# EntityOfCode/eoc-tfhe

Measured on AMD Instinct MI355X. Metric: gate bootstraps/sec (HomNAND), higher is better.
Workload: dtype f64

## Files before the change

eoc_tfhe_amd/__init__.py:

```python
import ctypes as C
import os

import numpy as np

_HERE = os.path.dirname(os.path.abspath(__file__))
LIB_PATH = os.environ.get("EOC_TFHE_LIB") or os.path.join(_HERE, "libeoc_tfhe_gpu.so")
N = 1024

OPS = dict(NAND=0, AND=1, OR=2, NOR=3, XOR=4, XNOR=5, ANDNY=6, ANDYN=7, ORNY=8, ORYN=9,
           MUX=10, NOT=11, COPY=12, CONST0=13, CONST1=14,
           MAJ=15, XOR3=16)


class EocError(RuntimeError):
    pass


class Params(C.Structure):
    _fields_ = [("n", C.c_int32), ("l", C.c_int32), ("Bgbit", C.c_int32), ("ks_t", C.c_int32),
                ("ks_basebit", C.c_int32), ("ks_stdev", C.c_double), ("bk_stdev", C.c_double)]

    def copy(self):
        q = Params()
        C.memmove(C.byref(q), C.byref(self), C.sizeof(Params))
# ... 96 lines not shown
        "eoc_decrypt_ints": (C.c_int, [vp, C.c_int, vp, sz, vp]),
        "eoc_lut_test_polynomial": (C.c_int, [C.c_int, vp, vp]),
        "eoc_lut_batch": (C.c_int, [C.c_int, vp, sz, vp, vp, sz]),
        "eoc_lut_many_test_polynomial": (C.c_int, [C.c_int, C.c_int, vp, vp]),
        "eoc_lut_many_batch_device": (C.c_int, [vp, C.c_int, vp, sz, vp, vp, sz, vp]),
        "eoc_lut_many_batch": (C.c_int, [C.c_int, C.c_int, vp, sz, vp, vp, sz]),
        "eoc_global_encrypt_ints": (C.c_int, [C.c_int, vp, sz, vp]),
        "eoc_global_decrypt_ints": (C.c_int, [C.c_int, vp, sz, vp]),
        "eoc_engine_stats": (C.c_int, [vp, C.POINTER(u64 * 3)]),
        "eoc_stats": (C.c_int, [C.POINTER(u64 * 3)]),
        "eoc_gpu_init": (C.c_int, [C.c_int, PP]),
        "eoc_gpu_init_multi": (C.c_int, [vp, C.c_int, PP]),
        "eoc_gpu_init_from_env": (C.c_int, [PP]),
        "eoc_gpu_set_devices": (C.c_int, [C.POINTER(C.c_int), C.c_int]),
        "eoc_gpu_engine_count": (C.c_int, []),
        "eoc_global_engine_at": (vp, [C.c_int]),
        "eoc_upload_cloud_key_arrays": (C.c_int, [vp, vp]),
        "eoc_stats_multi": (C.c_int, [vp, C.c_int, C.POINTER(C.c_double)]),
        "eoc_key_broadcast_method": (C.c_char_p, []),
        "eoc_host_path_buffer_grows": (u64, []),
        "eoc_rccl_origin": (C.c_char_p, []),
        "eoc_rccl_selftest": (C.c_int, [C.c_int, sz]),
        "eoc_worker_wakeups": (u64, [C.c_int]),
        "eoc_shard_range": (None, [sz, C.c_int, C.c_int, C.POINTER(sz), C.POINTER(sz)]),
        "eoc_gate_batch_submit": (C.c_int, [C.c_int, vp, vp, vp, vp, vp, sz, C.POINTER(u64)]),
        "eoc_gate_batch_wait": (C.c_int, [u64]),
        "eoc_global_gate_batch_submit": (C.c_int, [C.c_int, vp, vp, vp, vp, vp, sz, C.POINTER(u64)]),
        "eoc_host_alloc": (vp, [sz]),
        "eoc_host_free": (None, [vp]),
        "eoc_engine_reserve": (C.c_int, [vp, sz, sz, sz]),
        "eoc_engine_workspace_grows": (u64, [vp]),
        "eoc_engine_blind_rotate_launches": (u64, [vp]),
        "eoc_engine_blind_rotate_wide_launches": (u64, [vp]),
        "eoc_engine_resident_jobs": (C.c_size_t, [vp]),
        "eoc_engine_device": (C.c_int, [vp]),
        "eoc_engine_params": (PP, [vp]),
        "eoc_engine_adopt_cloud_key_device": (C.c_int, [vp, vp, vp]),
        "eoc_upload_cloud_key": (C.c_int, [vp]),
        "eoc_global_engine": (vp, []),
        "eoc_gpu_shutdown": (None, []),
        "eoc_gate_batch": (C.c_int, [C.c_int, vp, vp, vp, vp, vp, sz]),
        "eoc_circuit_run": (C.c_int, [vp, sz, vp, sz, sz]),
        "generateGateKey": (vp, [C.c_int, u64]),
        "resetGateKey": (None, []),
        "encryptBit": (vp, [C.c_int, C.c_char_p]),
        "decryptBit": (C.c_int, [C.c_char_p, C.c_char_p]),
        "constantBit": (vp, [C.c_int]),
        "gateNAND": (vp, [C.c_char_p, C.c_char_p, C.c_char_p]),
        "gateAND": (vp, [C.c_char_p, C.c_char_p, C.c_char_p]),
        "gateOR": (vp, [C.c_char_p, C.c_char_p, C.c_char_p]),
        "gateNOR": (vp, [C.c_char_p, C.c_char_p, C.c_char_p]),
        "gateXOR": (vp, [C.c_char_p, C.c_char_p, C.c_char_p]),
        "gateXNOR": (vp, [C.c_char_p, C.c_char_p, C.c_char_p]),
        "gateNOT": (vp, [C.c_char_p, C.c_char_p]),
        "gateMUX": (vp, [C.c_char_p, C.c_char_p, C.c_char_p, C.c_char_p]),
        "gateMAJ": (vp, [C.c_char_p, C.c_char_p, C.c_char_p, C.c_char_p]),
        "gateXOR3": (vp, [C.c_char_p, C.c_char_p, C.c_char_p, C.c_char_p]),
        "generateSecretKey": (vp, [C.c_char_p, C.c_char_p]),
        "generatePublicKey": (vp, []),
        "encryptInteger": (vp, [C.c_int32, C.c_char_p]),
        "encryptInteger_dummy": (vp, [C.c_int32, C.c_char_p]),
        "decryptInteger": (C.c_int, [C.c_char_p, C.c_char_p, C.c_char_p, C.c_char_p]),
        "addCiphertexts": (vp, [C.c_char_p, C.c_char_p, C.c_char_p]),
        "subtractCiphertexts": (vp, [C.c_char_p, C.c_char_p, C.c_char_p]),
        "encrypt8BitASCIIString": (vp, [C.c_char_p, C.c_int16, C.c_char_p]),
        "decrypt8BitASCIIString": (vp, [C.c_char_p, C.c_int16, C.c_char_p, C.c_char_p, C.c_char_p]),
# ... 369 lines not shown
        _check(self.L.eoc_circuit_run_device(self.h, C.addressof(arr), len(gates), d_wires, n_wires, instances, stream),
               "eoc_circuit_run_device")

    def fft_fwd_device(self, d_polys, d_specs, count, stream=None):
        _check(self.L.eoc_dbg_fft_fwd_device(self.h, d_polys, d_specs, count, stream), "eoc_dbg_fft_fwd_device")

    def fft_inv_device(self, d_specs, d_polys, count, stream=None):
        _check(self.L.eoc_dbg_fft_inv_device(self.h, d_specs, d_polys, count, stream), "eoc_dbg_fft_inv_device")

    def blind_rotate_device(self, d_t, d_u, count, stream=None):
        _check(self.L.eoc_blind_rotate_device(self.h, d_t, d_u, count, stream), "eoc_blind_rotate_device")

    def keyswitch_device(self, d_u, d_out, count, stream=None):
        _check(self.L.eoc_keyswitch_device(self.h, d_u, d_out, count, stream), "eoc_keyswitch_device")

    def lut_batch_device(self, d_tv, n_luts, d_in, d_out, count, stream=None):
        _check(self.L.eoc_lut_batch_device(self.h, d_tv, n_luts, d_in, d_out, count, stream), "eoc_lut_batch_device")

    def lut_many_batch_device(self, n_tables, d_tv, n_luts, d_in, d_out, count, stream=None):
        _check(self.L.eoc_lut_many_batch_device(self.h, int(n_tables), d_tv, n_luts, d_in, d_out, count, stream),
               "eoc_lut_many_batch_device")

    def compact_expand_device(self, d_lists, count, d_out, stream=None):
        _check(self.L.eoc_compact_expand_device(self.h, d_lists, count, d_out, stream), "eoc_compact_expand_device")

    def resident_jobs(self):
        return int(self.L.eoc_engine_resident_jobs(self.h))

    def stats(self):
        out = (C.c_uint64 * 3)()
        _check(self.L.eoc_engine_stats(self.h, C.byref(out)), "eoc_engine_stats")
        return dict(batches=out[0], bootstraps=out[1], keyswitches=out[2],
                    br_launches=int(self.L.eoc_engine_blind_rotate_launches(self.h)),
                    br_wide_launches=int(self.L.eoc_engine_blind_rotate_wide_launches(self.h)))


def circuit_bootstraps(gates):
    arr = (Gate * len(gates))(*gates)
    return lib().eoc_circuit_bootstraps(C.addressof(arr), len(gates))


def netlist_optimize(gates, outputs, extension_gates=True):
    arr = (Gate * max(1, len(gates)))(*gates)
    out = (Gate * max(1, len(gates)))()
    outs = (C.c_int32 * max(1, len(outputs)))(*outputs)
    n = lib().eoc_netlist_optimize_ex(C.addressof(arr), len(gates), C.addressof(outs), len(outputs), C.addressof(out),
                                      0 if extension_gates else 1)
    if n < 0:
        raise EocError(f"eoc_netlist_optimize failed ({n}): not a single-assignment netlist?")
    return [Gate(out[k].op, out[k].in0, out[k].in1, out[k].in2, out[k].out) for k in range(n)]


def netlist_levels(gates):
    arr = (Gate * max(1, len(gates)))(*gates)
    lev = (C.c_int32 * max(1, len(gates)))()
    depth = C.c_int64(0)
    n = lib().eoc_netlist_levels(C.addressof(arr), len(gates), C.addressof(lev), C.addressof(depth))
    if n < 0:
        raise EocError(f"eoc_netlist_levels failed ({n})")
    return list(lev[:len(gates)]), int(n), int(depth.value)


def netlist_cost(gates, instances, resident_jobs=0):
    arr = (Gate * max(1, len(gates)))(*gates)
    c = lib().eoc_netlist_cost(C.addressof(arr), len(gates), int(instances), int(resident_jobs))
    if c < 0:
        raise EocError(f"eoc_netlist_cost failed ({c})")
# ... 511 lines not shown
```

eoc_tfhe_amd/csrc/engine.hip:

```cpp
#include "kernels.hip.h"
#include "canon_twiddles.h"
#include "common.h"
#include "../../include/eoc_tfhe_gpu.h"

#include <algorithm>
#include <cstdio>
#include <cstdlib>
#include <cstring>
#include <mutex>
#include <new>
#include <vector>

using namespace eoc;

#define HIP_TRY(expr)                                                                       \
    do {                                                                                    \
        hipError_t _e = (expr);                                                             \
        if (_e != hipSuccess) {                                                             \
            eoc_set_error("%s failed: %s (%s:%d)", #expr, hipGetErrorString(_e), __FILE__, \
                          __LINE__);                                                        \
            return EOC_ERR_HIP;                                                             \
        }                                                                                   \
    } while (0)

struct eoc_engine {
    int device = 0;
    eoc_params p{};
    int kpl = 0;
    size_t n1p = 0;
    d2 *d_tw = nullptr, *d_twist = nullptr;
    double *d_bkfft = nullptr;
    int32_t *d_ksk = nullptr;
    bool own_keys = false;
    const double *bkfft = nullptr;
    const int32_t *ksk = nullptr;
    struct Workspace {
        uint16_t *d_bara = nullptr;
        int32_t *d_u = nullptr;
        uint32_t *d_ubar = nullptr;
        int32_t *d_acc_state = nullptr;
        size_t ws_jobs = 0;
        GateDesc *d_descs = nullptr, *h_descs = nullptr;
        size_t ws_descs = 0, desc_pos = 0;
        hipEvent_t ring_ev = nullptr;
        bool ring_ev_set = false;
        bool ring_pushed_since_mark = false;
        GateDesc *d_persist = nullptr, *h_persist = nullptr;
        size_t persist_cap = 0, persist_pos = 0;
        int32_t *d_mixed = nullptr;
        uint32_t *h_perm = nullptr;
        hipEvent_t perm_ev = nullptr;
        size_t ws_mixed = 0;
    } ws;
    unsigned long long *d_stamps = nullptr;
    int num_cus = 256;
    int prio_duty_override = INT32_MIN;
    int prio_multi = -1;
    int br_slice = 0;
    bool no_fold = false;
    bool scalar_abar = false;
    bool no_pool = false;
    int br_parts = 0;
    int br_wide = -1;
    int bara_stride = 0;
    bool ks_waves_ok = true;
    uint64_t stats[3] = {0, 0, 0};
    uint64_t ws_grows = 0;
    uint64_t br_launches = 0;
    uint64_t br_wide_launches = 0;
    bool profiling = false;
    struct Span { hipEvent_t a, b; int kind; };
    std::vector<Span> spans;
    double kernel_ms[3] = {0, 0, 0};
    uint64_t kernel_launches[3] = {0, 0, 0};
    std::mutex mu;
};

enum { KIND_PREPARE = 0, KIND_BLIND_ROTATE = 1, KIND_KEYSWITCH = 2 };

struct SpanGuard {
    eoc_engine *e;
    hipStream_t st;
    hipEvent_t a = nullptr, b = nullptr;
    int kind;
    SpanGuard(eoc_engine *e_, hipStream_t st_, int kind_) : e(e_), st(st_), kind(kind_)
    {
        if (!e->profiling) return;
        if (hipEventCreate(&a) != hipSuccess || hipEventCreate(&b) != hipSuccess) {
            a = b = nullptr;
            return;
        }
        hipEventRecord(a, st);
    }
    ~SpanGuard()
    {
        if (!a) return;
        hipEventRecord(b, st);
        e->spans.push_back({a, b, kind});
    }
};

static int valid_params(const eoc_params *p)
// ... 86 lines not shown
                      "-- the FP64 external product is not exact beyond that --, ks_t * ks_basebit <= 31, ks_basebit <= 4)");
        return EOC_ERR_ARG;
    }
    int cnt = eoc_device_count();
    if (cnt <= 0 || device < 0 || device >= cnt) {
        eoc_set_error("eoc_engine_create: no usable HIP device (count=%d, asked %d); the gate path has no CPU fallback",
                      cnt, device);
        return EOC_ERR_NO_DEVICE;
    }
    HIP_TRY(hipSetDevice(device));
    eoc_engine *e = new (std::nothrow) eoc_engine();
    if (!e) return EOC_ERR_ALLOC;
    e->device = device;
    e->p = *p;
    e->kpl = 2 * p->l;
    e->n1p = eoc_ksk_row_stride(p);
    e->bara_stride = (p->n + 1 + 31) / 32 * 32;
    int rc = upload_tables(e);
    if (rc) {
        delete e;
        return rc;
    }
    {
        int cus = 0;
        if (hipDeviceGetAttribute(&cus, hipDeviceAttributeMultiprocessorCount, device) == hipSuccess && cus > 0) e->num_cus = cus;
        if (const char *s = getenv("EOC_TFHE_PRIO_DUTY")) e->prio_duty_override = atoi(s);
        if (const char *s = getenv("EOC_TFHE_PRIO_MULTI")) e->prio_multi = atoi(s);
        if (const char *s = getenv("EOC_TFHE_BR_SLICE")) e->br_slice = atoi(s);
        if (getenv("EOC_TFHE_NO_FOLD")) e->no_fold = true;
        if (getenv("EOC_TFHE_NO_POOL")) e->no_pool = true;
        if (const char *s = getenv("EOC_TFHE_SCALAR_ABAR")) e->scalar_abar = atoi(s) != 0;
        if (const char *s = getenv("EOC_TFHE_BR_PARTS")) e->br_parts = atoi(s);
        if (const char *s = getenv("EOC_TFHE_BR_WIDE")) e->br_wide = atoi(s);
    }
#define EOC_KS_ATTR(TT, NWV, IWV)                                                                              \
    if (hipFuncSetAttribute(reinterpret_cast<const void *>(&k_keyswitch_waves<TT, NWV, IWV>),                  \
                            hipFuncAttributeMaxDynamicSharedMemorySize, KS3Cfg<TT, NWV, IWV>::LDS_BYTES) != hipSuccess) \
        e->ks_waves_ok = false
    EOC_KS_ATTR(8, 8, 16);
    EOC_KS_ATTR(8, 8, 32);
    EOC_KS_ATTR(8, 4, 64);
    EOC_KS_ATTR(8, 8, 64);
#undef EOC_KS_ATTR
    if (!e->ks_waves_ok) (void)hipGetLastError();
    *out = e;
    return EOC_OK;
}

static void free_ws(eoc_engine::Workspace &W)
{
    hipFree(W.d_bara);
    hipFree(W.d_u);
    hipFree(W.d_ubar);
    hipFree(W.d_acc_state);
    hipFree(W.d_descs);
    hipFree(W.d_mixed);
    if (W.h_descs) hipHostFree(W.h_descs);
    if (W.h_perm) hipHostFree(W.h_perm);
    if (W.perm_ev) hipEventDestroy(W.perm_ev);
    if (W.ring_ev) hipEventDestroy(W.ring_ev);
    hipFree(W.d_persist);
    if (W.h_persist) hipHostFree(W.h_persist);
    W = eoc_engine::Workspace();
}

extern "C" void eoc_engine_destroy(eoc_engine *e)
{
    if (!e) return;
    hipSetDevice(e->device);
    hipDeviceSynchronize();
    hipFree(e->d_tw);
    hipFree(e->d_twist);
    if (e->own_keys) {
        hipFree(e->d_bkfft);
        hipFree(e->d_ksk);
    }
    free_ws(e->ws);
    hipFree(e->d_stamps);
    delete e;
}

static bool stream_is_capturing(hipStream_t st)
{
    hipStreamCaptureStatus cap = hipStreamCaptureStatusNone;
    return st && hipStreamIsCapturing(st, &cap) == hipSuccess && cap == hipStreamCaptureStatusActive;
}

static int ensure_ws(eoc_engine *e, eoc_engine::Workspace &W, size_t jobs, size_t descs, size_t mixed, hipStream_t st = nullptr)
{
    if (jobs <= W.ws_jobs && descs <= W.ws_descs && mixed <= W.ws_mixed) return EOC_OK;
    if (stream_is_capturing(st)) {
        eoc_set_error("graph capture: the workspace would have to grow (jobs %zu > %zu, descriptors %zu > %zu or mixed rows "
                      "%zu > %zu); call eoc_engine_reserve with the sizes of the captured work before capturing",
                      jobs, W.ws_jobs, descs, W.ws_descs, mixed, W.ws_mixed);
        return EOC_ERR_STATE;
    }
    HIP_TRY(hipDeviceSynchronize());
    if (jobs > W.ws_jobs) {
        hipFree(W.d_bara);
        hipFree(W.d_u);
        hipFree(W.d_ubar);
        W.d_bara = nullptr;
        W.d_u = nullptr;
        W.d_ubar = nullptr;
        W.ws_jobs = 0;
        size_t cap = (std::max<size_t>(jobs, 1024) + 63) / 64 * 64;
        HIP_TRY(hipMalloc(&W.d_bara, cap * e->bara_stride * sizeof(uint16_t)));
        HIP_TRY(hipMalloc(&W.d_u, cap * (kN + 1) * sizeof(int32_t)));
        HIP_TRY(hipMalloc(&W.d_ubar, (cap + KS_GT) * (size_t)kN * sizeof(uint32_t)));
// ... 114 lines not shown
    HIP_TRY(hipSetDevice(e->device));
    hipStream_t st = (hipStream_t)hip_stream;
    dim3 grid((unsigned)((count + 3) / 4));
    hipLaunchKernelGGL(k_fft_inv_polys, grid, dim3(256), 0, st, d_specs, d_polys, count, e->d_tw, e->d_twist);
    HIP_TRY(hipGetLastError());
    return EOC_OK;
}

static int build_cloud_key_images(eoc_engine *e, const int32_t *bk, const int32_t *ksk, double *d_bkfft,
                                  int32_t *d_ksk)
{
    const eoc_params &p = e->p;
    const size_t npoly = (size_t)p.n * e->kpl * 2;
    int32_t *d_bk = nullptr;
    HIP_TRY(hipMalloc(&d_bk, npoly * kN * 4));
    if (hipMemcpy(d_bk, bk, npoly * kN * 4, hipMemcpyHostToDevice) != hipSuccess) {
        hipFree(d_bk);
        eoc_set_error("cloud key upload failed");
        return EOC_ERR_HIP;
    }
    int rc = launch_fft_fwd(e, d_bk, d_bkfft, npoly, 0x1p-9, nullptr);
    hipError_t se = hipDeviceSynchronize();
    hipFree(d_bk);
    if (rc) return rc;
    HIP_TRY(se);
    const size_t rows = (size_t)kN * p.ks_t * (((size_t)1 << p.ks_basebit) - 1);
    HIP_TRY(hipMemset(d_ksk, 0, eoc_ksk_dev_bytes(&p)));
    HIP_TRY(hipMemcpy2D(d_ksk, e->n1p * 4, ksk, (size_t)(p.n + 1) * 4, (size_t)(p.n + 1) * 4, rows,
                        hipMemcpyHostToDevice));
    HIP_TRY(hipDeviceSynchronize());
    return EOC_OK;
}

extern "C" int eoc_engine_load_cloud_key(eoc_engine *e, const int32_t *bk, const int32_t *ksk)
{
    if (!e || !bk || !ksk) return EOC_ERR_ARG;
    std::lock_guard<std::mutex> g(e->mu);
    HIP_TRY(hipSetDevice(e->device));
    if (!e->own_keys) {
        HIP_TRY(hipMalloc(&e->d_bkfft, eoc_bkfft_bytes(&e->p)));
        HIP_TRY(hipMalloc(&e->d_ksk, eoc_ksk_dev_bytes(&e->p)));
        e->own_keys = true;
    }
    int rc = build_cloud_key_images(e, bk, ksk, e->d_bkfft, e->d_ksk);
    if (rc) return rc;
    e->bkfft = e->d_bkfft;
    e->ksk = e->d_ksk;
    return EOC_OK;
}

extern "C" int eoc_engine_build_cloud_key_device(eoc_engine *e, const int32_t *bk, const int32_t *ksk,
                                                 void *d_bkfft, void *d_ksk)
{
    if (!e || !bk || !ksk || !d_bkfft || !d_ksk) return EOC_ERR_ARG;
    std::lock_guard<std::mutex> g(e->mu);
    HIP_TRY(hipSetDevice(e->device));
    int rc = build_cloud_key_images(e, bk, ksk, static_cast<double *>(d_bkfft), static_cast<int32_t *>(d_ksk));
    if (rc) return rc;
    e->bkfft = static_cast<const double *>(d_bkfft);
    e->ksk = static_cast<const int32_t *>(d_ksk);
    return EOC_OK;
}

extern "C" int eoc_engine_set_cloud_key_device(eoc_engine *e, const void *d_bkfft, const void *d_ksk)
{
    if (!e || !d_bkfft || !d_ksk) return EOC_ERR_ARG;
    std::lock_guard<std::mutex> g(e->mu);
    e->bkfft = static_cast<const double *>(d_bkfft);
    e->ksk = static_cast<const int32_t *>(d_ksk);
    return EOC_OK;
}
extern "C" int eoc_engine_adopt_cloud_key_device(eoc_engine *e, void *d_bkfft, void *d_ksk)
{
    if (!e || !d_bkfft || !d_ksk) return EOC_ERR_ARG;
    std::lock_guard<std::mutex> g(e->mu);
    HIP_TRY(hipSetDevice(e->device));
    if (e->own_keys) {
        hipFree(e->d_bkfft);
        hipFree(e->d_ksk);
    }
    e->d_bkfft = static_cast<double *>(d_bkfft);
    e->d_ksk = static_cast<int32_t *>(d_ksk);
    e->own_keys = true;
    e->bkfft = e->d_bkfft;
    e->ksk = e->d_ksk;
    return EOC_OK;
}
extern "C" int eoc_engine_cloud_key_device(eoc_engine *e, const void **d_bkfft, const void **d_ksk)
{
    if (!e || !e->bkfft || !e->ksk) return EOC_ERR_NO_KEY;
    if (d_bkfft) *d_bkfft = e->bkfft;
    if (d_ksk) *d_ksk = e->ksk;
    return EOC_OK;
}

typedef eoc_engine::Workspace WS;

struct BRWork {
    uint32_t njobs = 0;
    enum Seed { GATE, TV, MANY } seed = GATE;
    const int32_t *tv = nullptr;
    uint32_t tv_rows = 1, n_tables = 0;
    enum Fold { NONE, KS, KS_AND_PREP } fold = NONE;
    const GateDesc *descs = nullptr, *inline_desc = nullptr;
    uint32_t S = 0;
};

struct BRSeg { uint32_t off, njobs; bool wide; };
struct BRPlan {
    std::vector<BRSeg> segs;
    int parts;
};
static BRPlan plan_blind_rotate(uint32_t njobs_total, int num_cus, int l, int kpl, int n, int br_slice, int br_parts, int br_wide)
{
    const uint32_t resident_pair = 4u * (uint32_t)num_cus, resident_wide = 8u * (uint32_t)num_cus;
    const bool can_wide = l == 2 && br_wide != 0;
    const bool force_wide = can_wide && br_wide > 0;
    const int auto_parts = kpl * 2 * kNH * 16 > 80 * 1024 ? 2 : 1;
    BRPlan plan;
// ... 79 lines not shown
    else if (l == 3 && Bgbit == 7) fn = br_pair_kernel<3, 7>(seed, sabar);
    else if (l == 1) fn = br_pair_kernel<1, 0>(seed, sabar);
    else if (l == 2) fn = br_pair_kernel<2, 0>(seed, sabar);
    else if (l == 3) fn = br_pair_kernel<3, 0>(seed, sabar);
    else if (l == 4) fn = br_pair_kernel<4, 0>(seed, sabar);
    return {fn, dim3(njobs), dim3(128), kBRLds};
}

static int launch_blind_rotate(eoc_engine *e, WS &W, const BRWork &w, hipStream_t st)
{
    const bool folds = w.fold != BRWork::NONE;
    if ((w.seed != BRWork::GATE && !w.tv) || (w.seed == BRWork::MANY && (folds || w.n_tables == 0)) ||
        (folds && !w.inline_desc && (!w.descs || !w.S)) || (w.inline_desc && (w.fold != BRWork::KS_AND_PREP || !w.S))) {
        eoc_set_error("internal: blind rotation of family %d with fold %d: a table family needs its test polynomials, the "
                      "many-LUT kernel has no fold, a fold needs descriptors and their row count", (int)w.seed, (int)w.fold);
        return EOC_ERR_STATE;
    }
    SpanGuard span(e, st, KIND_BLIND_ROTATE);
    const BRPlan plan = plan_blind_rotate(w.njobs, e->num_cus, e->p.l, e->kpl, e->p.n, e->br_slice, e->br_parts, e->br_wide);
    for (const BRSeg &sg : plan.segs) {
        const BRKernel k = blind_rotate_kernel(sg.wide, e->p.l, e->p.Bgbit, e->scalar_abar, w.seed, sg.njobs);
        if (!k.fn) return EOC_ERR_ARG;
        for (int part = 0; part < plan.parts; part++) {
            BRArgs a = blind_rotate_args(e, W, w, sg, part, plan.parts);
            void *args[] = {&a, (void *)&e->d_tw, (void *)&e->d_twist, (void *)&w.tv, (void *)&w.tv_rows, (void *)&w.n_tables};
            HIP_TRY(hipLaunchKernel(k.fn, k.grid, k.block, args, k.lds, st));
            e->br_launches++;
            e->br_wide_launches += sg.wide;
        }
    }
    return EOC_OK;
}

static int launch_keyswitch(eoc_engine *e, WS &W, const GateDesc *d_descs, uint32_t ngates, uint32_t S, hipStream_t st,
                            bool init_done, const GateDesc *inline_desc)
{
    KSArgs a;
    a.inline_desc = inline_desc != nullptr;
    if (inline_desc) a.desc0 = *inline_desc;
    else a.desc0 = GateDesc{0, 0, nullptr, nullptr, nullptr, nullptr};
    a.ksk = e->ksk;
    a.u = W.d_u;
    a.ubar = W.d_ubar;
    a.n = e->p.n;
    a.n1p = (int)e->n1p;
    a.t = e->p.ks_t;
    a.basebit = e->p.ks_basebit;
    a.S = S;
    a.mu = (int32_t)(1u << 29);
    SpanGuard span(e, st, KIND_KEYSWITCH);
    if (!init_done) {
        hipLaunchKernelGGL(k_ks_init, dim3(S, ngates), dim3(256), 0, st, d_descs, a);
        HIP_TRY(hipGetLastError());
    }
    const uint32_t ntiles = (S + KS_GT - 1) / KS_GT;
    const int ncb = (int)(e->n1p / 64);
    const int bb = e->p.ks_basebit, t = e->p.ks_t;
#define EOC_KS_LAUNCH(TT, NWV, IWV)                                                                     \
    do {                                                                                                  \
        auto kfn = k_keyswitch_waves<TT, NWV, IWV>;                                                       \
        constexpr int lds = KS3Cfg<TT, NWV, IWV>::LDS_BYTES;                                              \
        constexpr int ns = KS3Cfg<TT, NWV, IWV>::NS;                                                      \
        hipLaunchKernelGGL(kfn, dim3(ntiles * (unsigned)ncb * ns, ngates), dim3(64 * NWV), lds, st, d_descs, a); \
    } while (0)
    const bool fast = bb == 2 && t == 8 && e->ks_waves_ok;
    if (fast && ncb == 4) EOC_KS_LAUNCH(8, 8, 16);
    else if (fast && ncb == 8) EOC_KS_LAUNCH(8, 8, 32);
    else if (fast && ncb == 12) EOC_KS_LAUNCH(8, 4, 64);
    else if (fast && ncb == 16) EOC_KS_LAUNCH(8, 8, 64);
    else
        hipLaunchKernelGGL(k_keyswitch_generic, dim3(S, ngates), dim3(256), 0, st, d_descs, a);
#undef EOC_KS_LAUNCH
    HIP_TRY(hipGetLastError());
    return EOC_OK;
}

static inline bool op_const(int op) { return op == OP_CONST0 || op == OP_CONST1; }
static inline bool op_free(int op) { return op == OP_NOT || op == OP_COPY || op_const(op); }
static inline bool op_valid(int op) { return (op >= 0 && op <= OP_XOR3); }
static inline bool op_lin3(int op) { return op == OP_MAJ || op == OP_XOR3; }
static inline int op_inputs(int op) { return op_const(op) ? 0 : (op_free(op) ? 1 : (op == OP_MUX || op_lin3(op) ? 3 : 2)); }

constexpr size_t kMaxGatesPerLaunch = 32768;

static int push_descs(WS &W, const GateDesc *src, size_t count, hipStream_t st, GateDesc **d_out)
{
    if (stream_is_capturing(st)) {
        if (W.persist_pos + count > W.persist_cap) {
            eoc_set_error("graph capture: descriptor arena exhausted (%zu of %zu used, %zu wanted); "
                          "eoc_engine_reserve a larger max_descs before capturing", W.persist_pos, W.persist_cap, count);
            return EOC_ERR_STATE;
        }
        memcpy(W.h_persist + W.persist_pos, src, count * sizeof(GateDesc));
        HIP_TRY(hipMemcpyAsync(W.d_persist + W.persist_pos, W.h_persist + W.persist_pos, count * sizeof(GateDesc),
                               hipMemcpyHostToDevice, st));
        *d_out = W.d_persist + W.persist_pos;
        W.persist_pos += count;
        return EOC_OK;
    }
// ... 573 lines not shown
            e->kernel_ms[i] = 0;
            e->kernel_launches[i] = 0;
        }
    }
    return EOC_OK;
}

#ifdef EOC_STAMPS
extern "C" int eoc_dbg_stamps(eoc_engine *e, size_t waves, unsigned long long *host_out)
{
    if (!e) return EOC_ERR_ARG;
    HIP_TRY(hipSetDevice(e->device));
    if (!host_out) {
        hipFree(e->d_stamps);
        HIP_TRY(hipMalloc(&e->d_stamps, waves * 16 * 8));
        HIP_TRY(hipMemset(e->d_stamps, 0, waves * 16 * 8));
        return EOC_OK;
    }
    HIP_TRY(hipDeviceSynchronize());
    HIP_TRY(hipMemcpy(host_out, e->d_stamps, waves * 16 * 8, hipMemcpyDeviceToHost));
    return EOC_OK;
}
#endif

extern "C" int eoc_engine_stats(eoc_engine *e, uint64_t out[3])
{
    if (!e || !out) return EOC_ERR_ARG;
    for (int i = 0; i < 3; i++) out[i] = e->stats[i];
    return EOC_OK;
}
extern "C" uint64_t eoc_engine_workspace_grows(eoc_engine *e) { return e ? e->ws_grows : 0; }
extern "C" uint64_t eoc_engine_blind_rotate_launches(eoc_engine *e) { return e ? e->br_launches : 0; }
extern "C" uint64_t eoc_engine_blind_rotate_wide_launches(eoc_engine *e) { return e ? e->br_wide_launches : 0; }
extern "C" size_t eoc_engine_resident_jobs(eoc_engine *e)
{
    if (!e) return 0;
    const bool wide = e->p.l == 2 && e->br_wide != 0;
    return (size_t)(wide ? 8 : 4) * (size_t)e->num_cus;
}
extern "C" int eoc_engine_device(eoc_engine *e) { return e ? e->device : -1; }
extern "C" const eoc_params *eoc_engine_params(eoc_engine *e) { return e ? &e->p : nullptr; }
```

eoc_tfhe_amd/csrc/kernels.hip.h:

```cpp
#pragma once
#include <hip/hip_runtime.h>
#include <stdint.h>
#include <type_traits>

namespace eoc {

typedef double d2 __attribute__((ext_vector_type(2)));

constexpr int kN = 1024;
constexpr int kNH = 512;
constexpr int kScr = 568;
constexpr int kTwF1 = 0;
constexpr int kTwF2 = 32;
constexpr int kTwI1 = 32 + 256;
constexpr int kTwI0 = 32 + 256 + 32;
constexpr int kTwEntries = 32 + 256 + 32 + 256;

#define EOC_FMA(a, b, c) __builtin_fma((a), (b), (c))

#define EOC_SQRT_HALF 0x1.6a09e667f3bcdp-1
#define EOC_E128_RE 0x1.d906bcf328d46p-1
#define EOC_E128_IM 0x1.87de2a6aea963p-2
#define EOC_E64_RE 0x1.f6297cff75cb0p-1
#define EOC_E64_IM 0x1.8f8b83c69a60bp-3
// ... 863 lines not shown
        int *r = s_all + lane * C::ROWI;
#pragma unroll
        for (int c = 0; c < 16; c++) *reinterpret_cast<i4 *>(r + 4 * c) = acc[c];
    }
    __syncthreads();
    const int col = (int)cb * 64 + lane;
#pragma unroll 4
    for (int k = 0; k < 64 / NWV; k++) {
        const int ct = w * (64 / NWV) + k;
        const int v = s_all[ct * C::ROWI + lane];
        if (v != 0 && s0 + ct < A.S && col <= A.n) atomicAdd(d.out + (size_t)(s0 + ct) * (A.n + 1) + col, v);
    }
}

__global__ __launch_bounds__(256) void k_keyswitch_generic(const GateDesc *__restrict__ descs, KSArgs A)
{
    const GateDesc d = A.inline_desc ? A.desc0 : descs[blockIdx.y];
    const uint32_t s = blockIdx.x, job = d.job_base + s;
    const int base1 = (1 << A.basebit) - 1;
    int32_t *o = d.out + (size_t)s * (A.n + 1);
    for (int m = threadIdx.x; m <= A.n; m += 256) {
        uint32_t acc = (uint32_t)o[m];
        for (int i = 0; i < kN; i++) {
            const uint32_t ub = A.ubar[(size_t)job * kN + i];
            for (int j = 0; j < A.t; j++) {
                const uint32_t dg = (ub >> (32 - (j + 1) * A.basebit)) & (uint32_t)base1;
                if (dg) acc -= (uint32_t)A.ksk[(((size_t)i * A.t + j) * base1 + (dg - 1)) * A.n1p + m];
            }
        }
        o[m] = (int32_t)acc;
    }
}

constexpr int kCompactSlotsPerWG = 16;
__global__ __launch_bounds__(256) void k_compact_expand(const int32_t *__restrict__ lists, uint64_t first, uint32_t S,
                                                        uint32_t *__restrict__ ubar, int32_t *__restrict__ out, int n,
                                                        uint32_t prec_offset)
{
    static_assert(kN % kCompactSlotsPerWG == 0, "a workgroup's slots lie inside one list");
    __shared__ int32_t s_c0[kN];
    const uint64_t g0 = (first / kCompactSlotsPerWG + blockIdx.x) * kCompactSlotsPerWG;
    const int32_t *list = lists + (g0 / kN) * (uint64_t)(2 * kN);
    for (int k = threadIdx.x; k < kN; k += 256) s_c0[k] = list[k];
    __syncthreads();
    for (int q = 0; q < kCompactSlotsPerWG; q++) {
        const uint64_t g = g0 + q;
        if (g < first || g >= first + S) continue;
        const uint32_t s = (uint32_t)(g - first);
        const int j = (int)(g % kN);
        uint32_t *row = ubar + (size_t)s * kN;
        for (int i = threadIdx.x; i < kN; i += 256) {
            const uint32_t v = (uint32_t)s_c0[(j - i) & (kN - 1)];
            row[i] = (i <= j ? v : 0u - v) + prec_offset;
        }
        int32_t *o = out + (size_t)s * (n + 1);
        for (int m = threadIdx.x; m < n; m += 256) o[m] = 0;
        if (threadIdx.x == 0) o[n] = list[kN + j];
    }
}

}
```

include/eoc_tfhe_gpu.h:

```cpp
#ifndef EOC_TFHE_GPU_H
#define EOC_TFHE_GPU_H
#include <stddef.h>
#include <stdint.h>

#ifdef __cplusplus
extern "C" {
#endif

#define EOC_N 1024

typedef struct eoc_params {
    int32_t n;
    int32_t l;
    int32_t Bgbit;
    int32_t ks_t;
    int32_t ks_basebit;
    double ks_stdev;
    double bk_stdev;
} eoc_params;

enum eoc_op {
    EOC_NAND = 0, EOC_AND = 1, EOC_OR = 2, EOC_NOR = 3, EOC_XOR = 4, EOC_XNOR = 5,
    EOC_ANDNY = 6, EOC_ANDYN = 7, EOC_ORNY = 8, EOC_ORYN = 9, EOC_MUX = 10,
    EOC_NOT = 11, EOC_COPY = 12,
// ... 40 lines not shown
int32_t eoc_lwe_phase(const eoc_secret_key *sk, const int32_t *ct);
int eoc_host_threads(void);
int32_t eoc_modswitch_to_torus32(int32_t mu, int32_t Msize);
int32_t eoc_modswitch_from_torus32(int32_t phase, int32_t Msize);

typedef struct eoc_engine eoc_engine;

int eoc_device_count(void);
int eoc_engine_create(int device, const eoc_params *p, eoc_engine **out);
void eoc_engine_destroy(eoc_engine *e);
const char *eoc_last_error(void);

int eoc_device_alloc(eoc_engine *e, size_t bytes, void **d_ptr);
int eoc_device_free(eoc_engine *e, void *d_ptr);
int eoc_host_to_device(eoc_engine *e, void *d_dst, const void *src, size_t bytes);
int eoc_device_to_host(eoc_engine *e, void *dst, const void *d_src, size_t bytes);
int eoc_engine_synchronize(eoc_engine *e);

size_t eoc_bkfft_bytes(const eoc_params *p);
size_t eoc_ksk_dev_bytes(const eoc_params *p);
size_t eoc_ksk_row_stride(const eoc_params *p);

int eoc_engine_load_cloud_key(eoc_engine *e, const int32_t *bk, const int32_t *ksk);
int eoc_engine_build_cloud_key_device(eoc_engine *e, const int32_t *bk, const int32_t *ksk,
                                      void *d_bkfft, void *d_ksk);
int eoc_engine_set_cloud_key_device(eoc_engine *e, const void *d_bkfft, const void *d_ksk);
int eoc_engine_adopt_cloud_key_device(eoc_engine *e, void *d_bkfft, void *d_ksk);
int eoc_engine_cloud_key_device(eoc_engine *e, const void **d_bkfft, const void **d_ksk);

int eoc_engine_reserve(eoc_engine *e, size_t max_jobs, size_t max_descs, size_t max_mixed_rows);
uint64_t eoc_engine_workspace_grows(eoc_engine *e);
uint64_t eoc_engine_blind_rotate_launches(eoc_engine *e);
uint64_t eoc_engine_blind_rotate_wide_launches(eoc_engine *e);
size_t eoc_engine_resident_jobs(eoc_engine *e);
int eoc_engine_device(eoc_engine *e);
const eoc_params *eoc_engine_params(eoc_engine *e);
int eoc_gate_batch_device(eoc_engine *e, int op, const uint8_t *ops, const int32_t *d_in0,
                          const int32_t *d_in1, const int32_t *d_in2, int32_t *d_out, size_t count,
                          void *hip_stream);

typedef struct eoc_gate {
    int32_t op;
    int32_t in0, in1, in2;
    int32_t out;
} eoc_gate;
int eoc_circuit_run_device(eoc_engine *e, const eoc_gate *gates, size_t n_gates, int32_t *d_wires,
                           size_t n_wires, size_t instances, void *hip_stream);
size_t eoc_circuit_bootstraps(const eoc_gate *gates, size_t n_gates);
int64_t eoc_netlist_optimize(const eoc_gate *gates, size_t n_gates, const int32_t *outputs, size_t n_outputs,
                             eoc_gate *gates_out);
enum { EOC_NL_BOOTS_GATES_ONLY = 1 };
int64_t eoc_netlist_optimize_ex(const eoc_gate *gates, size_t n_gates, const int32_t *outputs, size_t n_outputs,
                                eoc_gate *gates_out, unsigned flags);
int64_t eoc_netlist_levels(const eoc_gate *gates, size_t n_gates, int32_t *level_of, int64_t *bootstrap_levels);
int64_t eoc_netlist_cost(const eoc_gate *gates, size_t n_gates, size_t instances, size_t resident_jobs);

int eoc_dbg_fft_fwd_device(eoc_engine *e, const int32_t *d_polys, double *d_specs, size_t count,
                           void *hip_stream);
int eoc_dbg_fft_inv_device(eoc_engine *e, const double *d_specs, int32_t *d_polys, size_t count,
                           void *hip_stream);
int eoc_blind_rotate_device(eoc_engine *e, const int32_t *d_t, int32_t *d_u, size_t count,
                            void *hip_stream);
int eoc_keyswitch_device(eoc_engine *e, const int32_t *d_u, int32_t *d_out, size_t count,
                         void *hip_stream);
int eoc_lut_batch_device(eoc_engine *e, const int32_t *d_tv, size_t n_luts, const int32_t *d_in, int32_t *d_out,
                         size_t count, void *hip_stream);
// ... 117 lines not shown
```

Baseline: 338,100.

## Add MFMA int8 keyswitch kernel using byte-limb decomposed key-switching key

```diff
diff --git a/eoc_tfhe_amd/__init__.py b/eoc_tfhe_amd/__init__.py
--- a/eoc_tfhe_amd/__init__.py
+++ b/eoc_tfhe_amd/__init__.py
@@ -152,6 +152,7 @@
         "eoc_engine_workspace_grows": (u64, [vp]),
         "eoc_engine_blind_rotate_launches": (u64, [vp]),
         "eoc_engine_blind_rotate_wide_launches": (u64, [vp]),
+        "eoc_engine_keyswitch_mfma_launches": (u64, [vp]),
         "eoc_engine_resident_jobs": (C.c_size_t, [vp]),
         "eoc_engine_device": (C.c_int, [vp]),
         "eoc_engine_params": (PP, [vp]),
@@ -587,7 +588,8 @@
         _check(self.L.eoc_engine_stats(self.h, C.byref(out)), "eoc_engine_stats")
         return dict(batches=out[0], bootstraps=out[1], keyswitches=out[2],
                     br_launches=int(self.L.eoc_engine_blind_rotate_launches(self.h)),
-                    br_wide_launches=int(self.L.eoc_engine_blind_rotate_wide_launches(self.h)))
+                    br_wide_launches=int(self.L.eoc_engine_blind_rotate_wide_launches(self.h)),
+                    ks_mfma_launches=int(self.L.eoc_engine_keyswitch_mfma_launches(self.h)))
 
 
 def circuit_bootstraps(gates):
diff --git a/eoc_tfhe_amd/csrc/engine.hip b/eoc_tfhe_amd/csrc/engine.hip
--- a/eoc_tfhe_amd/csrc/engine.hip
+++ b/eoc_tfhe_amd/csrc/engine.hip
@@ -34,6 +34,8 @@
     bool own_keys = false;
     const double *bkfft = nullptr;
     const int32_t *ksk = nullptr;
+    void *d_ksl = nullptr;
+    bool ksl_ready = false;
     struct Workspace {
         uint16_t *d_bara = nullptr;
         int32_t *d_u = nullptr;
@@ -64,10 +66,12 @@
     int br_wide = -1;
     int bara_stride = 0;
     bool ks_waves_ok = true;
+    int ks_mfma = -1;
     uint64_t stats[3] = {0, 0, 0};
     uint64_t ws_grows = 0;
     uint64_t br_launches = 0;
     uint64_t br_wide_launches = 0;
+    uint64_t ks_mfma_launches = 0;
     bool profiling = false;
     struct Span { hipEvent_t a, b; int kind; };
     std::vector<Span> spans;
@@ -220,6 +224,7 @@
         if (const char *s = getenv("EOC_TFHE_SCALAR_ABAR")) e->scalar_abar = atoi(s) != 0;
         if (const char *s = getenv("EOC_TFHE_BR_PARTS")) e->br_parts = atoi(s);
         if (const char *s = getenv("EOC_TFHE_BR_WIDE")) e->br_wide = atoi(s);
+        if (const char *s = getenv("EOC_TFHE_KS_MFMA")) e->ks_mfma = atoi(s) != 0;
     }
 #define EOC_KS_ATTR(TT, NWV, IWV)                                                                              \
     if (hipFuncSetAttribute(reinterpret_cast<const void *>(&k_keyswitch_waves<TT, NWV, IWV>),                  \
@@ -263,6 +268,7 @@
         hipFree(e->d_bkfft);
         hipFree(e->d_ksk);
     }
+    hipFree(e->d_ksl);
     free_ws(e->ws);
     hipFree(e->d_stamps);
     delete e;
@@ -443,6 +449,19 @@
     return EOC_OK;
 }
 
+static int install_ks_limbs(eoc_engine *e)
+{
+    e->ksl_ready = false;
+    if (e->p.ks_basebit != 2 || e->p.ks_t != 8 || e->ks_mfma == 0) return EOC_OK;
+    if (!e->d_ksl) HIP_TRY(hipMalloc(&e->d_ksl, ks_limb_bytes((int)e->n1p)));
+    HIP_TRY(hipDeviceSynchronize());
+    ks_limbs_launch(e->ksk, e->d_ksl, (int)e->n1p, nullptr);
+    HIP_TRY(hipGetLastError());
+    HIP_TRY(hipDeviceSynchronize());
+    e->ksl_ready = true;
+    return EOC_OK;
+}
+
 extern "C" int eoc_engine_load_cloud_key(eoc_engine *e, const int32_t *bk, const int32_t *ksk)
 {
     if (!e || !bk || !ksk) return EOC_ERR_ARG;
@@ -457,7 +476,7 @@
     if (rc) return rc;
     e->bkfft = e->d_bkfft;
     e->ksk = e->d_ksk;
-    return EOC_OK;
+    return install_ks_limbs(e);
 }
 
 extern "C" int eoc_engine_build_cloud_key_device(eoc_engine *e, const int32_t *bk, const int32_t *ksk,
@@ -470,16 +489,17 @@
     if (rc) return rc;
     e->bkfft = static_cast<const double *>(d_bkfft);
     e->ksk = static_cast<const int32_t *>(d_ksk);
-    return EOC_OK;
+    return install_ks_limbs(e);
 }
 
 extern "C" int eoc_engine_set_cloud_key_device(eoc_engine *e, const void *d_bkfft, const void *d_ksk)
 {
     if (!e || !d_bkfft || !d_ksk) return EOC_ERR_ARG;
     std::lock_guard<std::mutex> g(e->mu);
+    HIP_TRY(hipSetDevice(e->device));
     e->bkfft = static_cast<const double *>(d_bkfft);
     e->ksk = static_cast<const int32_t *>(d_ksk);
-    return EOC_OK;
+    return install_ks_limbs(e);
 }
 extern "C" int eoc_engine_adopt_cloud_key_device(eoc_engine *e, void *d_bkfft, void *d_ksk)
 {
@@ -495,7 +515,7 @@
     e->own_keys = true;
     e->bkfft = e->d_bkfft;
     e->ksk = e->d_ksk;
-    return EOC_OK;
+    return install_ks_limbs(e);
 }
 extern "C" int eoc_engine_cloud_key_device(eoc_engine *e, const void **d_bkfft, const void **d_ksk)
 {
@@ -641,6 +661,7 @@
     return EOC_OK;
 }
 
+constexpr uint32_t kKsMfmaMinS = 1;
 static int launch_keyswitch(eoc_engine *e, WS &W, const GateDesc *d_descs, uint32_t ngates, uint32_t S, hipStream_t st,
                             bool init_done, const GateDesc *inline_desc)
 {
@@ -673,7 +694,12 @@
         hipLaunchKernelGGL(kfn, dim3(ntiles * (unsigned)ncb * ns, ngates), dim3(64 * NWV), lds, st, d_descs, a); \
     } while (0)
     const bool fast = bb == 2 && t == 8 && e->ks_waves_ok;
-    if (fast && ncb == 4) EOC_KS_LAUNCH(8, 8, 16);
+    const bool mfma = bb == 2 && t == 8 && e->ksl_ready && (e->ks_mfma == 1 || (e->ks_mfma < 0 && S >= kKsMfmaMinS));
+    if (mfma) {
+        ks_mfma_launch(ks_mfma_plan(S, (int)e->n1p), ngates, d_descs, a, e->d_ksl, st);
+        e->ks_mfma_launches++;
+    }
+    else if (fast && ncb == 4) EOC_KS_LAUNCH(8, 8, 16);
     else if (fast && ncb == 8) EOC_KS_LAUNCH(8, 8, 32);
     else if (fast && ncb == 12) EOC_KS_LAUNCH(8, 4, 64);
     else if (fast && ncb == 16) EOC_KS_LAUNCH(8, 8, 64);
@@ -1313,6 +1339,7 @@
 extern "C" uint64_t eoc_engine_workspace_grows(eoc_engine *e) { return e ? e->ws_grows : 0; }
 extern "C" uint64_t eoc_engine_blind_rotate_launches(eoc_engine *e) { return e ? e->br_launches : 0; }
 extern "C" uint64_t eoc_engine_blind_rotate_wide_launches(eoc_engine *e) { return e ? e->br_wide_launches : 0; }
+extern "C" uint64_t eoc_engine_keyswitch_mfma_launches(eoc_engine *e) { return e ? e->ks_mfma_launches : 0; }
 extern "C" size_t eoc_engine_resident_jobs(eoc_engine *e)
 {
     if (!e) return 0;
diff --git a/eoc_tfhe_amd/csrc/kernels.hip.h b/eoc_tfhe_amd/csrc/kernels.hip.h
--- a/eoc_tfhe_amd/csrc/kernels.hip.h
+++ b/eoc_tfhe_amd/csrc/kernels.hip.h
@@ -919,6 +919,160 @@
     }
 }
 
+typedef int i16 __attribute__((ext_vector_type(16)));
+constexpr int KSM_KI = 4;
+
+template <int NWV>
+__global__ __launch_bounds__(64 * NWV, 2) void k_keyswitch_mfma(const GateDesc *__restrict__ descs, KSArgs A,
+                                                                 const i4 *__restrict__ limbs, int nsl)
+{
+    constexpr int MT = 64 * NWV;
+    constexpr int CHUNKS = KSM_KI * 4;
+    constexpr int NLD = CHUNKS / NWV;
+    static_assert(CHUNKS % NWV == 0, "shape");
+    __shared__ i4 s_b[2][CHUNKS * 64];
+
+    const GateDesc d = A.inline_desc ? A.desc0 : descs[blockIdx.y];
+    const uint32_t ntiles = (A.S + MT - 1) / MT, nct = (uint32_t)A.n1p / 32u;
+    const uint32_t tile = blockIdx.x % ntiles, rest = blockIdx.x / ntiles;
+    const uint32_t ct = rest % nct, slice = rest / nct;
+    const int per = kN / nsl, nstage = per / KSM_KI;
+    const int ibeg = (int)slice * per;
+    const int tid = threadIdx.x, lane = tid & 63, r = lane & 31, h = lane >> 5;
+    const int w = __builtin_amdgcn_readfirstlane(tid >> 6);
+    const uint32_t row0 = tile * MT + (uint32_t)w * 64u;
+
+    typedef uint32_t u4 __attribute__((ext_vector_type(4)));
+    const u4 *ubp[2];
+#pragma unroll
+    for (int m = 0; m < 2; m++) {
+        const uint32_t s = row0 + 32u * m + r;
+        const uint32_t job = d.job_base + (s < A.S ? s : A.S - 1);
+        ubp[m] = reinterpret_cast<const u4 *>(A.ubar + (size_t)job * kN + ibeg);
+    }
+    const i4 *bsrc = limbs + ((size_t)ibeg * nct + ct) * 256 + lane;
+    i4 stg[NLD];
+    auto stage_load = [&](int st) {
+#pragma unroll
+        for (int x = 0; x < NLD; x++) {
+            const int c = w + NWV * x;
+            stg[x] = bsrc[((size_t)(st * KSM_KI + (c >> 2)) * nct) * 256 + (c & 3) * 64];
+        }
+    };
+    auto stage_store = [&](int buf) {
+#pragma unroll
+        for (int x = 0; x < NLD; x++) s_b[buf][(w + NWV * x) * 64 + lane] = stg[x];
+    };
+
+    i16 acc[2][4];
+#pragma unroll
+    for (int m = 0; m < 2; m++)
+#pragma unroll
+        for (int k = 0; k < 4; k++)
+#pragma unroll
+            for (int q = 0; q < 16; q++) acc[m][k][q] = 0;
+
+    stage_load(0);
+    u4 ubc[2] = {ubp[0][0], ubp[1][0]};
+    stage_store(0);
+    stage_load(nstage > 1 ? 1 : 0);
+    __syncthreads();
+    const int sh0 = 27 - 8 * h;
+#pragma unroll 1
+    for (int st = 0; st < nstage; st++) {
+        const int buf = st & 1;
+        const int stn = st + 1 < nstage ? st + 1 : st;
+        const u4 ubn[2] = {ubp[0][stn], ubp[1][stn]};
+#pragma unroll
+        for (int ki = 0; ki < KSM_KI; ki++) {
+            i4 b[4], a[2];
+#pragma unroll
+            for (int k = 0; k < 4; k++) b[k] = s_b[buf][(ki * 4 + k) * 64 + lane];
+#pragma unroll
+            for (int m = 0; m < 2; m++) {
+                const uint32_t ub = ubc[m][ki];
+#pragma unroll
+                for (int q = 0; q < 4; q++) a[m][q] = (int)(1u << ((ub >> (sh0 - 2 * q)) & 24u));
+            }
+#pragma unroll
+            for (int m = 0; m < 2; m++)
+#pragma unroll
+                for (int k = 0; k < 4; k++)
+                    acc[m][k] = __builtin_amdgcn_mfma_i32_32x32x32_i8(a[m], b[k], acc[m][k], 0, 0, 0);
+        }
+        stage_store(buf ^ 1);
+        stage_load(st + 2 < nstage ? st + 2 : nstage - 1);
+        __syncthreads();
+        ubc[0] = ubn[0];
+        ubc[1] = ubn[1];
+    }
+
+    const int col = (int)ct * 32 + r;
+    if (col <= A.n) {
+#pragma unroll
+        for (int m = 0; m < 2; m++)
+#pragma unroll
+            for (int q = 0; q < 16; q++) {
+                const uint32_t s = row0 + 32u * m + (uint32_t)((q & 3) + 8 * (q >> 2) + 4 * h);
+                const uint32_t v = (uint32_t)acc[m][0][q] + ((uint32_t)acc[m][1][q] << 8) + ((uint32_t)acc[m][2][q] << 16) +
+                                   ((uint32_t)acc[m][3][q] << 24);
+                if (v != 0 && s < A.S) atomicAdd(d.out + (size_t)s * (A.n + 1) + col, (int)(0u - v));
+            }
+    }
+}
+
+__global__ __launch_bounds__(256) void k_ksk_limbs(const int32_t *__restrict__ ksk, uint32_t *__restrict__ limbs, int n1p)
+{
+    const uint32_t nct = (uint32_t)n1p / 32u;
+    const uint32_t limb = blockIdx.x & 3u, ct = (blockIdx.x >> 2) % nct, i = (blockIdx.x >> 2) / nct;
+    const int q = threadIdx.x & 3, lane = threadIdx.x >> 2, r = lane & 31, h = lane >> 5;
+    const int j = 4 * h + q;
+    const int32_t *row = ksk + ((size_t)i * 8 + j) * 3 * n1p + ct * 32 + r;
+    uint32_t o = 0;
+#pragma unroll
+    for (int dg = 1; dg <= 3; dg++) {
+        int32_t v = row[(size_t)(dg - 1) * n1p];
+        int32_t l = 0;
+        for (uint32_t k = 0; k <= limb; k++) {
+            l = (int32_t)(((uint32_t)v + 128u) & 255u) - 128;
+            v = (int32_t)((uint32_t)v - (uint32_t)l) >> 8;
+        }
+        o |= ((uint32_t)l & 255u) << (8 * dg);
+    }
+    limbs[(size_t)blockIdx.x * 256 + threadIdx.x] = o;
+}
+
+static inline size_t ks_limb_bytes(int n1p) { return (size_t)kN * (size_t)(n1p / 32) * 4096; }
+static inline void ks_limbs_launch(const int32_t *ksk, void *limbs, int n1p, hipStream_t st)
+{
+    hipLaunchKernelGGL(k_ksk_limbs, dim3((unsigned)(kN * (n1p / 32) * 4)), dim3(256), 0, st, ksk,
+                       static_cast<uint32_t *>(limbs), n1p);
+}
+
+struct KSMPlan {
+    int nwv, nsl;
+    unsigned gx;
+};
+static inline KSMPlan ks_mfma_plan(uint32_t S, int n1p)
+{
+    KSMPlan p;
+    p.nwv = 4;
+    const unsigned ntiles = (S + 64 * p.nwv - 1) / (64 * p.nwv), nct = (unsigned)n1p / 32u;
+    p.nsl = 1;
+    while (p.nsl < 32 && ntiles * nct * p.nsl * p.nwv < 2048u) p.nsl *= 2;
+    p.gx = ntiles * nct * (unsigned)p.nsl;
+    return p;
+}
+static inline void ks_mfma_launch(const KSMPlan &pl, uint32_t ngates, const GateDesc *descs, const KSArgs &a,
+                                  const void *limbs, hipStream_t st)
+{
+    const i4 *lp = static_cast<const i4 *>(limbs);
+    if (pl.nwv == 8)
+        hipLaunchKernelGGL(k_keyswitch_mfma<8>, dim3(pl.gx, ngates), dim3(512), 0, st, descs, a, lp, pl.nsl);
+    else
+        hipLaunchKernelGGL(k_keyswitch_mfma<4>, dim3(pl.gx, ngates), dim3(256), 0, st, descs, a, lp, pl.nsl);
+}
+
 constexpr int kCompactSlotsPerWG = 16;
 __global__ __launch_bounds__(256) void k_compact_expand(const int32_t *__restrict__ lists, uint64_t first, uint32_t S,
                                                         uint32_t *__restrict__ ubar, int32_t *__restrict__ out, int n,
diff --git a/include/eoc_tfhe_gpu.h b/include/eoc_tfhe_gpu.h
--- a/include/eoc_tfhe_gpu.h
+++ b/include/eoc_tfhe_gpu.h
@@ -96,6 +96,7 @@
 uint64_t eoc_engine_workspace_grows(eoc_engine *e);
 uint64_t eoc_engine_blind_rotate_launches(eoc_engine *e);
 uint64_t eoc_engine_blind_rotate_wide_launches(eoc_engine *e);
+uint64_t eoc_engine_keyswitch_mfma_launches(eoc_engine *e);
 size_t eoc_engine_resident_jobs(eoc_engine *e);
 int eoc_engine_device(eoc_engine *e);
 const eoc_params *eoc_engine_params(eoc_engine *e);
```

Result: faster. 344,800, median of 6 (+2.0%).
